# SJTU-ViSYS-team/VisFly

Hardware: AMD Instinct MI355X
Metric: agent-steps/sec (dynamics.step, visual=False) (higher is better)
Workload: dtype f32

## Files before the change

### visfly_amd/csrc/vf_common.hpp

```cpp
#pragma once
#include <hip/hip_runtime.h>

#include <cstdarg>
#include <cstdio>
#include <cstdlib>

#include "visfly_amd.h"

namespace vf {

char* err_buf();

inline int fail(int code, const char* fmt, ...)
{
    va_list ap;
    va_start(ap, fmt);
    vsnprintf(err_buf(), 512, fmt, ap);
    va_end(ap);
    return code;
}

#ifdef VF_CHAIN_PLUGIN
#define VF_HIP(expr)                                                                        \
    do {                                                                                    \
        hipError_t e_ = (expr);                                                             \
        if (e_ != hipSuccess) return -1000 - (int)e_;                                       \
    } while (0)
#else
#define VF_HIP(expr)                                                                        \
    do {                                                                                    \
        hipError_t e_ = (expr);                                                             \
        if (e_ != hipSuccess)                                                               \
            return vf::fail(VF_EHIP, "%s failed: %s (%s:%d)", #expr, hipGetErrorString(e_), \
                            __FILE__, __LINE__);                                            \
    } while (0)
#endif

inline hipStream_t as_stream(vf_stream_t s) { return reinterpret_cast<hipStream_t>(s); }

constexpr int kBlock = 256;

inline int blocks_for(int n) { return (n + kBlock - 1) / kBlock; }

inline int grid_for(long n, int cap = 512)
{
    long b = (n + kBlock - 1) / kBlock;
    return (int)(b < 1 ? 1 : (b > cap ? cap : b));
}

inline bool use_split(int agents_padded, const vf_dyn_cfg& cfg)
{
    if (cfg.action_type != VF_ACT_THRUST && cfg.action_type != VF_ACT_BODYRATE) return false;
    return agents_padded <= 32768;
}

struct vf_env_dev {
    vf_env_cfg cfg;
    unsigned agent0;
    float hit_y;
};

#ifdef __HIPCC__
__device__ __forceinline__ unsigned env_agent0(const vf_env_cfg& e) { return reinterpret_cast<const vf_env_dev&>(e).agent0; }
__device__ __forceinline__ float env_hit_y(const vf_env_cfg& e) { return reinterpret_cast<const vf_env_dev&>(e).hit_y; }

__device__ __forceinline__ double wave_sum(double x)
{
#pragma unroll
    for (int o = 32; o > 0; o >>= 1) x += __shfl_down(x, o, 64);
    return x;
}
__device__ __forceinline__ float wave_sumf(float x)
{
#pragma unroll
    for (int o = 32; o > 0; o >>= 1) x += __shfl_down(x, o, 64);
    return x;
}

struct U4 {
    unsigned x, y, z, w;
};

__device__ __forceinline__ U4 philox4x32_10(U4 ctr, unsigned k0, unsigned k1)
{
#pragma unroll
    for (int r = 0; r < 10; ++r) {
        const unsigned hi0 = __umulhi(0xD2511F53u, ctr.x), lo0 = 0xD2511F53u * ctr.x;
        const unsigned hi1 = __umulhi(0xCD9E8D57u, ctr.z), lo1 = 0xCD9E8D57u * ctr.z;
        ctr = U4{hi1 ^ ctr.y ^ k0, lo1, hi0 ^ ctr.w ^ k1, lo0};
        k0 += 0x9E3779B9u;
        k1 += 0xBB67AE85u;
    }
    return ctr;
}

__device__ __forceinline__ float u01(unsigned x) { return (float)(x & 0xFFFFFFu) * (1.0f / 16777216.0f); }

constexpr unsigned kTagPpoNoise = 0xac7u, kTagRowNoise = 0xb977u;

__device__ __forceinline__ void philox_normal4(unsigned row, unsigned long long step, unsigned tag, unsigned long long seed, float* e)
{
    const U4 r = philox4x32_10(U4{row, (unsigned)step, (unsigned)(step >> 32), tag}, (unsigned)seed, (unsigned)(seed >> 32));
    const float u1 = ((float)(r.x >> 8) + 1.0f) * (1.0f / 16777216.0f), u2 = (float)(r.y >> 8) * (1.0f / 16777216.0f);
    const float u3 = ((float)(r.z >> 8) + 1.0f) * (1.0f / 16777216.0f), u4 = (float)(r.w >> 8) * (1.0f / 16777216.0f);
    const float ra = sqrtf(-2.0f * logf(u1)), rb = sqrtf(-2.0f * logf(u3));
    const float two_pi = 6.28318530717958647692f;
    e[0] = ra * cosf(two_pi * u2); e[1] = ra * sinf(two_pi * u2); e[2] = rb * cosf(two_pi * u4); e[3] = rb * sinf(two_pi * u4);
}

__device__ __forceinline__ float act_fwd(float z, int kind)
{
    switch (kind) {
    case VF_ACTIVATION_RELU: return z > 0.0f ? z : 0.0f;
// ... 123 lines not shown
```

### visfly_amd/csrc/vf_dyn_device.hpp

```cpp
#pragma once
#include <hip/hip_runtime.h>

#include "vf_common.hpp"
#include "vf_pair_algebra.hpp"
#include "vf_step_consts.hpp"
#include "vf_xmath.hpp"
#include "visfly_amd.h"

#pragma clang fp contract(off)

namespace vf {

struct Agent {
    float p[3];
    Quat q;
    float v[3];
    float w[3];
    float wm[4];
    float T[4];
    float aa[3];
    float acc[3];
    float t;
    float wnd[3];
};


__device__ __forceinline__ float clampf(float v, float lo, float hi)
{
    float r = v < lo ? lo : v;
    return r > hi ? hi : r;
}

struct RotorK {
    vf_f2 K0, K1;
};
__device__ __forceinline__ RotorK rotor_k(const vf_dyn_cfg& c)
{
    RotorK k{pair_of(c.c_motor, c.tm0), pair_of(c.tm1, c.tm2)};
    keep_in_vgprs(k.K0);
    keep_in_vgprs(k.K1);
    return k;
}

struct IntervalMats {
    Mat4P B;
    Mat3P J, Jinv;
    RotorK k;
};
__device__ __forceinline__ IntervalMats interval_mats(const vf_dyn_cfg& c)
{
    return IntervalMats{mat4_pairs(c.B), mat3_pairs(c.J), mat3_pairs(c.Jinv), rotor_k(c)};
}

struct MatsOfCfg {
    static constexpr bool paired_sqrt = false;
    __device__ __forceinline__ IntervalMats operator()(const vf_dyn_cfg& c) const { return interval_mats(c); }
};
struct StepConstsV {
    float4 v[8];
};
__device__ __forceinline__ StepConstsV load_step_consts(const vf_dyn_cfg* cp)
{
    unsigned z;
    asm("v_mov_b32 %0, 0" : "=v"(z));
    const float4* p = reinterpret_cast<const float4*>(reinterpret_cast<const char*>(cp) + kStepConstsOffset + z);
    StepConstsV k;
#pragma unroll
    for (int j = 0; j < 8; ++j) k.v[j] = p[j];
    return k;
}
struct MatsOfBlock {
    static constexpr bool paired_sqrt = true;
    StepConstsV k;
    __device__ __forceinline__ IntervalMats operator()(const vf_dyn_cfg& c) const
    {
        IntervalMats M;
#pragma unroll
        for (int j = 0; j < 4; ++j) {
            M.B.c01[j] = pair_of(k.v[j].x, k.v[j].y);
            M.B.c23[j] = pair_of(k.v[j].z, k.v[j].w);
        }
        const vf_f2 h[8] = {pair_of(k.v[4].x, k.v[4].y), pair_of(k.v[4].z, k.v[4].w), pair_of(k.v[5].x, k.v[5].y), pair_of(k.v[5].z, k.v[5].w),
                            pair_of(k.v[6].x, k.v[6].y), pair_of(k.v[6].z, k.v[6].w), pair_of(k.v[7].x, k.v[7].y), pair_of(k.v[7].z, k.v[7].w)};
#pragma unroll
        for (int j = 0; j < 3; ++j) {
            M.J.r0[j] = c.J[j];
            M.Jinv.r0[j] = c.Jinv[j];
            M.J.c12[j] = h[j];
            M.Jinv.c12[j] = h[3 + j];
        }
        M.k.K0 = h[6];
        M.k.K1 = h[7];
#pragma unroll
        for (int j = 0; j < 4; ++j) { keep_in_vgprs(M.B.c01[j]); keep_in_vgprs(M.B.c23[j]); }
#pragma unroll
        for (int j = 0; j < 3; ++j) { keep_in_vgprs(M.J.c12[j]); keep_in_vgprs(M.Jinv.c12[j]); }
        keep_in_vgprs(M.k.K0);
        keep_in_vgprs(M.k.K1);
        return M;
    }
};

struct Vec3P {
    float x;
    vf_f2 yz;
};

__device__ __forceinline__ void derivs(const IntervalMats& M, const QuatP& q, const QuatP& wq, const vf_f2 ft01, const vf_f2 ft23,
                                       QuatP& dq, Vec3P& dw)
{
    const QuatP p = qmul_p<false, false>(q, wq);
    const vf_f2 half = {0.5f, 0.5f};
    dq.wx = p.wx * half;
    dq.yz = p.yz * half;
    float Jw0;
    vf_f2 Jw12;
    mat3_p(M.J, wq.wx, wq.yz, Jw0, Jw12);
    const float w0 = wq.wx[1], w1 = wq.yz[0], w2 = wq.yz[1];
    const float c0 = __builtin_fmaf(w1, Jw12[1], -(w2 * Jw12[0]));
    const float c1 = __builtin_fmaf(w2, Jw0, -(w0 * Jw12[1]));
    const float c2 = __builtin_fmaf(w0, Jw12[0], -(w1 * Jw0));
    vf_f2 d0p = ft01;
    d0p[1] = ft01[1] - c0;
    const vf_f2 d12 = {ft23[0] - c1, ft23[1] - c2};
    mat3_p(M.Jinv, d0p, d12, dw.x, dw.yz);
}
// ... 397 lines not shown
struct NoCheckpoint {
    __device__ __forceinline__ void head(int, const Agent&) const {}
    __device__ __forceinline__ void end(const Agent&) const {}
};

struct RotorsP {
    vf_f2 Td[2], wd[2], wm[2], T[2];
    __device__ __forceinline__ RotorsP(const Agent& s, const float* Td_, const float* wd_)
    {
#pragma unroll
        for (int h = 0; h < 2; ++h) {
            Td[h] = pair_of(Td_[2 * h], Td_[2 * h + 1]);
            wd[h] = pair_of(wd_[2 * h], wd_[2 * h + 1]);
            wm[h] = pair_of(s.wm[2 * h], s.wm[2 * h + 1]);
            T[h] = pair_of(s.T[2 * h], s.T[2 * h + 1]);
        }
    }
    __device__ __forceinline__ void store(Agent& s) const
    {
#pragma unroll
        for (int h = 0; h < 2; ++h) {
            s.wm[2 * h] = wm[h][0]; s.wm[2 * h + 1] = wm[h][1];
            s.T[2 * h] = T[h][0]; s.T[2 * h + 1] = T[h][1];
        }
    }
};

template <int ACT, int INTEG, bool CTRL_DELAY, class CK = NoCheckpoint>
__device__ __forceinline__ void control_interval(const vf_dyn_cfg& c, Agent& s, const float* a,
                                                 const float* kl, const float* kq, bool vstrided = false, const CK& ck = CK{})
{
    float Td[4], wd[4];
    desired_thrusts<ACT>(c, s, a, Td, vstrided);
    rotor_setpoint<CTRL_DELAY>(c, Td, wd);
#pragma unroll 1
    for (int sub = 0; sub < c.interval_steps; ++sub) {
        ck.head(sub, s);
        float ft[4];
        motor_substep<CTRL_DELAY>(c, Td, wd, s.wm, s.T, ft);
        trans_substep<INTEG>(c, s.q, ft[0], kl, kq, s.wnd, s.p, s.v, s.acc);
        rot_substep<INTEG>(c, ft + 1, s.q, s.w, s.aa);
    }
    ck.end(s);
    finish_interval(c, s);
}

template <int ACT, int INTEG, bool CTRL_DELAY, class CK = NoCheckpoint, class MF = MatsOfCfg>
__device__ __forceinline__ void control_interval_pairs(const vf_dyn_cfg& c, Agent& s, const float* a,
                                                 const float* kl, const float* kq, bool vstrided = false, const CK& ck = CK{},
                                                 const MF& mf = MF{})
{
    float Td[4], wd[4];
    desired_thrusts<ACT>(c, s, a, Td, vstrided);
    rotor_setpoint<CTRL_DELAY, MF::paired_sqrt>(c, Td, wd);
    const IntervalMats M = mf(c);
    RotorsP r(s, Td, wd);
    QuatP q = to_pairs(s.q), wq{pair_of(0.0f, s.w[0]), pair_of(s.w[1], s.w[2])};
    const auto mirror = [&] {
        r.store(s);
        s.q = to_quat(q);
        s.w[0] = wq.wx[1]; s.w[1] = wq.yz[0]; s.w[2] = wq.yz[1];
    };
    const SubstepCfg sc = substep_cfg(c);
#pragma unroll 1
    for (int sub = 0; sub < sc.interval_steps; ++sub) {
        if constexpr (!__is_same(CK, NoCheckpoint)) {
            if (sub != 0) mirror();
            ck.head(sub, s);
        }
        vf_f2 ft01, ft23;
        motor_substep<CTRL_DELAY>(M.k, M.B, r.Td, r.wd, r.wm, r.T, ft01, ft23);
        trans_substep<INTEG>(sc, q, ft01[0], kl, kq, s.wnd, s.p, s.v, s.acc);
        rot_substep<INTEG>(sc, M, ft01, ft23, q, wq, s.aa);
    }
    mirror();
    ck.end(s);
    finish_interval(c, s);
}

typedef float vf_f4 __attribute__((ext_vector_type(4)));

template <int MODE>
__device__ __forceinline__ void st4_mode(float4* p, const float4 v)
{
    if constexpr (MODE == 0) {
        *p = v;
    } else {
        const vf_f4 x = {v.x, v.y, v.z, v.w};
        if constexpr (MODE == 1) asm volatile("global_store_dwordx4 %0, %1, off sc1" : : "v"(p), "v"(x) : "memory");
        else if constexpr (MODE == 2) asm volatile("global_store_dwordx4 %0, %1, off nt" : : "v"(p), "v"(x) : "memory");
        else asm volatile("global_store_dwordx4 %0, %1, off sc0 sc1" : : "v"(p), "v"(x) : "memory");
    }
}
template <int MODE>
__device__ __forceinline__ void st1_mode(float* p, const float v)
{
    if constexpr (MODE == 0) *p = v;
    else if constexpr (MODE == 1) asm volatile("global_store_dword %0, %1, off sc1" : : "v"(p), "v"(v) : "memory");
    else if constexpr (MODE == 2) asm volatile("global_store_dword %0, %1, off nt" : : "v"(p), "v"(v) : "memory");
    else asm volatile("global_store_dword %0, %1, off sc0 sc1" : : "v"(p), "v"(v) : "memory");
}

__device__ __forceinline__ float4* granule(float* __restrict__ S, int G, int i, int g)
{
    return reinterpret_cast<float4*>(S) + ((size_t)(i >> 6) * G + g) * VF_TILE + (i & 63);
}
// ... 249 lines not shown
```

### visfly_amd/csrc/vf_env.hip

```cpp
#include "vf_env_epilogue.hpp"

#pragma clang fp contract(off)

#ifdef VF_ENV_TRACE
__device__ unsigned long long* vf_env_trace_buf = nullptr;
__device__ unsigned vf_env_trace_cnt = 0, vf_env_trace_cap = 0;
extern "C" int vf_debug_env_trace(unsigned long long* buf, unsigned cap)
{
    unsigned zero = 0;
    if (hipMemcpyToSymbol(HIP_SYMBOL(vf_env_trace_buf), &buf, sizeof(buf)) != hipSuccess) return -1;
    if (hipMemcpyToSymbol(HIP_SYMBOL(vf_env_trace_cnt), &zero, sizeof(zero)) != hipSuccess) return -1;
    if (hipMemcpyToSymbol(HIP_SYMBOL(vf_env_trace_cap), &cap, sizeof(cap)) != hipSuccess) return -1;
    return 0;
}
#define VF_TR(i) tr[i] = __builtin_amdgcn_s_memrealtime()
#else
#define VF_TR(i)
#endif

namespace vf {

template <int KIND, int ACT, int INTEG, bool CTRL_DELAY, bool LAZY_SLOT = false, bool STRAIGHT = false>
__global__ __launch_bounds__(kBlock) void k_env_step(const vf_dyn_cfg* __restrict__ cp, const vf_env_cfg* __restrict__ ep, float* S,
                                                     const float4* action, int N, int G, int head, int helper, int delay_steps,
                                                     int g_drag, const EnvArgs g0)
{
    const vf_dyn_cfg& c = *cp;
    const vf_env_cfg& e = *ep;
    __shared__ __attribute__((aligned(16))) float tile[kBlock * 13];
    EnvArgs g = g0;
    g.d.S = S; g.d.action = action; g.d.N = N; g.d.G = G; g.d.head = head; g.helper = helper; g.d.g_drag = g_drag;
    if constexpr (STRAIGHT) {
        static_assert(!LAZY_SLOT, "the straight-line instance loads the spawn slot eagerly");
        g.d.g_drag = -1; g.d.wind = nullptr;
        g.out.done_list = nullptr; g.out.done_count = nullptr;
        g.stale = nullptr; g.auto_reset = 1;
        __builtin_assume(g.helper > 0);
        __builtin_assume(g.g_spawn_rd >= 0);
    }
    if (g.helper != 0 && (int)blockIdx.x >= g.helper) {
        const int nbm = g.helper;
        const int base = ((int)blockIdx.x - nbm) * kHelperSpan * kBlock + (int)threadIdx.x;
#pragma unroll 1
        for (int k = 0; k < kHelperSpan; ++k) spawn_helper(e, g, base + k * kBlock);
        return;
    }
#ifdef VF_ENV_TRACE
    unsigned long long tr[13];
#endif
    VF_TR(0);
    const int i = blockIdx.x * kBlock + threadIdx.x;
    const bool live = i < g.d.N;
    Agent s;
    Spares sp;
    float a[4], head_bits = 0.0f;
    ring_exchange_d(g.d, i, live, head_bits, a, nullptr, delay_steps);
    load_agent<false>(g.d.S, g.d.G, i, s, sp);
    float4 dk0 = make_float4(0.f, 0.f, 0.f, 0.f), dk1 = dk0;
    if (g.d.g_drag >= 0) { dk0 = *granule(g.d.S, g.d.G, i, g.d.g_drag); dk1 = *granule(g.d.S, g.d.G, i, g.d.g_drag + 1); }
    StepConstsV kv;
    if constexpr (STRAIGHT) kv = load_step_consts(cp);
#ifdef VF_ENV_TRACE
    VF_TR(1);
    prefetch_const_lines<(sizeof(vf_dyn_cfg) + 63) / 64, 2>(cp, ep, &ep->obs_mode);
    VF_TR(2);
    prefetch_kernarg<sizeof(EnvArgs) + 56>();
    VF_TR(3);
#else
    prefetch_kernarg_and_const_lines<sizeof(EnvArgs) + 56, (sizeof(vf_dyn_cfg) + 63) / 64, 2>(cp, ep, &ep->obs_mode);
#endif
    load_wind(c, g.d, i, live, s);
    if (delay_steps > 0) sp.vel = head_bits;
    float kl[3], kq[3];
    if (g.d.g_drag >= 0) {
        kl[0] = dk0.y; kl[1] = dk0.z; kl[2] = dk0.w;
        kq[0] = dk1.y; kq[1] = dk1.z; kq[2] = dk1.w;
    } else {
#pragma unroll
        for (int k = 0; k < 3; ++k) { kl[k] = c.k_lin[k]; kq[k] = c.k_quad[k]; }
    }
    if constexpr (STRAIGHT)
        asm("" : "+v"(s.wnd[0]), "+v"(s.wnd[1]), "+v"(s.wnd[2]), "+v"(kl[0]), "+v"(kl[1]), "+v"(kl[2]), "+v"(kq[0]), "+v"(kq[1]), "+v"(kq[2]));
#ifdef VF_ENV_TRACE
    asm volatile("s_waitcnt vmcnt(0)" ::: "memory");
    VF_TR(4);
    struct TraceCk {
        unsigned long long* tr;
        __device__ __forceinline__ void head(int sub, const Agent& s) const
        {
            if (sub < 2) { asm volatile("" :: "v"(s.wm[0]), "v"(s.q.w) : "memory"); tr[5 + sub] = __builtin_amdgcn_s_memrealtime(); }
        }
        __device__ __forceinline__ void end(const Agent&) const {}
    };
    control_interval_pairs<ACT, INTEG, CTRL_DELAY>(c, s, a, kl, kq, g.d.vstrided != 0, TraceCk{tr});
    asm volatile("" :: "v"(s.p[0]), "v"(s.q.w), "v"(s.v[0]), "v"(s.w[0]) : "memory");
    VF_TR(7);
#else
    if constexpr (STRAIGHT)
        control_interval_pairs<ACT, INTEG, CTRL_DELAY, NoCheckpoint, MatsOfBlock>(c, s, a, kl, kq, g.d.vstrided != 0, NoCheckpoint{}, MatsOfBlock{kv});
    else
        control_interval_pairs<ACT, INTEG, CTRL_DELAY>(c, s, a, kl, kq, g.d.vstrided != 0);
#endif
    const int wave = threadIdx.x >> 6;
#ifdef VF_ENV_TRACE
    env_epilogue<KIND, true, 1, false, LAZY_SLOT, STRAIGHT ? 7 : 0>(c, e, g, i, live, s, sp, blockIdx.x * kBlock + wave * 64, tile + wave * 64 * 13, nullptr, nullptr, tr);
    asm volatile("" ::: "memory");
    VF_TR(11);
    asm volatile("s_waitcnt vmcnt(0)" ::: "memory");
    VF_TR(12);
    if ((threadIdx.x & 63) == 0 && vf_env_trace_buf) {
        const unsigned slot = atomicAdd(&vf_env_trace_cnt, 1u);
        if (slot < vf_env_trace_cap) {
            unsigned long long* o = vf_env_trace_buf + (size_t)slot * 16;
            for (int k = 0; k < 13; ++k) o[k] = tr[k];
            o[13] = ((unsigned long long)blockIdx.x << 8) | wave;
            unsigned xcc = 0;
            asm volatile("s_getreg_b32 %0, hwreg(HW_REG_XCC_ID)" : "=s"(xcc));
            unsigned hwid = 0;
            asm volatile("s_getreg_b32 %0, hwreg(HW_REG_HW_ID)" : "=s"(hwid));
            o[14] = ((unsigned long long)xcc << 32) | hwid;
        }
    }
#else
    env_epilogue<KIND, true, 1, false, LAZY_SLOT, STRAIGHT ? 7 : 0>(c, e, g, i, live, s, sp, blockIdx.x * kBlock + wave * 64, tile + wave * 64 * 13);
#endif
}



template <int KIND>
__global__ __launch_bounds__(kBlock) void k_env_finish(const vf_dyn_cfg* __restrict__ cp, const vf_env_cfg* __restrict__ ep, const EnvArgs g)
{
    const vf_dyn_cfg& c = *cp;
    const vf_env_cfg& e = *ep;
    __shared__ __attribute__((aligned(16))) float tile[kBlock * 13];
    const int i = blockIdx.x * kBlock + threadIdx.x;
    const bool live = i < g.d.N;
    Agent s;
    Spares sp;
    load_agent<false>(g.d.S, g.d.G, i, s, sp);
    load_wind(c, g.d, i, live, s);
    const int wave = threadIdx.x >> 6;
    env_epilogue<KIND, true, 1, true>(c, e, g, i, live, s, sp, blockIdx.x * kBlock + wave * 64, tile + wave * 64 * 13);
}

template <int KIND, int ACT, int INTEG, bool CTRL_DELAY>
__global__ __launch_bounds__(kBlock) void k_env_rollout(const vf_dyn_cfg* __restrict__ cp, const vf_env_cfg* __restrict__ ep, const EnvArgs g0)
{
    const vf_dyn_cfg& c = *cp;
    const vf_env_cfg& e = *ep;
    __shared__ __attribute__((aligned(16))) float tile[kBlock * 13];
    const int i = blockIdx.x * kBlock + threadIdx.x;
    const int wave = threadIdx.x >> 6;
    EnvArgs g = g0;
    const bool live = i < g.d.N;
    Agent s;
    Spares sp;
    float a[4], head_bits = 0.0f;
    ring_exchange(c, g.d, i, live, head_bits, a);
    load_agent<false>(g.d.S, g.d.G, i, s, sp);
    load_wind(c, g.d, i, live, s);
    for (int k = 0;;) {
        if (c.delay_steps > 0) sp.vel = head_bits;
        float kl[3], kq[3];
        drag_of(c, g.d, i, kl, kq);
        control_interval_pairs<ACT, INTEG, CTRL_DELAY>(c, s, a, kl, kq, g.d.vstrided != 0);
        env_epilogue<KIND, false>(c, e, g, i, live, s, sp, blockIdx.x * kBlock + wave * 64, tile + wave * 64 * 13);
        if (++k >= g.K) break;
        g.d.action += g.action_stride;
        g.out.obs += g.obs_stride;
        g.out.reward += g.reward_stride;
        g.out.done += g.done_stride;
        g.d.head = g.d.head + 1 == c.delay_steps ? 0 : g.d.head + 1;
        ring_exchange(c, g.d, i, live, head_bits, a);
    }
    store_agent(g.d.S, g.d.G, i, s, sp);
}
// ... 612 lines not shown
```

### visfly_amd/csrc/vf_env_epilogue.hpp

```cpp
#pragma once
#include "vf_env_device.hpp"
#include "vf_handles.hpp"

#pragma clang fp contract(off)

namespace vf {

struct EnvArgs {
    DynArgs d;
    vf_env_out out;
    int g_race;
    int auto_reset;
    int K = 1;
    long long action_stride = 0, obs_stride = 0, reward_stride = 0, done_stride = 0;
    const float* ext_point = nullptr;
    const unsigned char* ext_oob = nullptr;
    int g_spawn_rd = -1, g_spawn_wr = -1, helper = 0;
    unsigned long long* stale = nullptr;
    int n_tiles = 0, stale_wr = 0;
};

struct EnvRegs {
    int step_count;
    float rewards;
// ... 14 lines not shown
__device__ __forceinline__ int set_flag(int flags, int bit, bool on) { return on ? (flags | bit) : (flags & ~bit); }

__device__ __forceinline__ int collision_flags(int flags, const Collision& col)
{
    flags = set_flag(flags, VF_F_COLLISION, col.hit);
    flags = set_flag(flags, VF_F_OUT_BOUNDS, col.oob);
    if (col.hit) flags |= VF_F_ONCE_COLLIDED;
    return flags;
}

struct SpawnSlot {
    float4 g0, g1, g2, g3;
};

#ifndef VF_HELPER_SPAN
#define VF_HELPER_SPAN 1
#endif
constexpr int kHelperSpan = VF_HELPER_SPAN;

__device__ __forceinline__ void spawn_helper(const vf_env_cfg& e, const EnvArgs& g, int i)
{
    if (i >= g.d.N) return;
    unsigned long long* word = nullptr;
    if (g.stale) {
        word = g.stale + (size_t)g.stale_wr * g.n_tiles + (i >> 6);
        if (!((*word >> (i & 63)) & 1ull)) return;
    }
    const unsigned need = ((unsigned)__float_as_int(granule(g.d.S, g.d.G, i, VF_G_ACC)->x) >> 8) + 1u;
    float4* dst = granule(g.d.S, g.d.G, i, g.g_spawn_wr);
    if (__float_as_uint(dst->x) != need) {
        Agent s;
        spawn_agent(e, env_agent0(e), i, need, true, s);
        const int gs = 64;
        dst[0] = make_float4(__uint_as_float(need), s.p[0], s.p[1], s.p[2]);
        dst[gs] = make_float4(s.q.w, s.q.x, s.q.y, s.q.z);
        dst[2 * gs] = make_float4(s.t, s.v[0], s.v[1], s.v[2]);
        dst[3 * gs] = make_float4(0.0f, s.w[0], s.w[1], s.w[2]);
    }
    if (word) atomicAnd(word, ~(1ull << (i & 63)));
}

__device__ __forceinline__ SpawnSlot load_spawn_slot(const EnvArgs& g, int i, bool wanted = true)
{
    const float4* src = granule(g.d.S, g.d.G, i, (wanted && g.g_spawn_rd >= 0) ? g.g_spawn_rd : 0);
    SpawnSlot slot;
    slot.g0 = src[0]; slot.g1 = src[64]; slot.g2 = src[128]; slot.g3 = src[192];
    return slot;
}

template <int KIND, bool STORE_STATE = true, int LANES = 1, bool EXT = false, bool LAZY_SLOT = false, int STRAIGHT = 0>
__device__ __forceinline__ void env_epilogue(const vf_dyn_cfg& c, const vf_env_cfg& e, const EnvArgs& g, int i, bool live,
                                             Agent& s, Spares& sp, int wave_first, float* tile, float* reward_reg = nullptr,
                                             bool* done_reg = nullptr, unsigned long long* tr = nullptr,
                                             int* gate_reg = nullptr)
{
#ifdef VF_ENV_TRACE
#define VF_EPI_TR(k, x) do { if (tr) { asm volatile("" :: "v"(x) : "memory"); tr[k] = __builtin_amdgcn_s_memrealtime(); } } while (0)
#else
#define VF_EPI_TR(k, x)
#endif
    EnvRegs er = unpack_env(sp);
    const float vel[3] = {s.v[0] + s.wnd[0], s.v[1] + s.wnd[1], s.v[2] + s.wnd[2]};
    constexpr bool NO_ROOT = (STRAIGHT & 4) && KIND == VF_ENV_HOVER && !EXT;
    Collision col = bbox_collision<NO_ROOT>(e, s.p);
    if constexpr (EXT) {
        if (g.ext_point && live) {
            const float* q = g.ext_point + 3 * (size_t)i;
#pragma unroll
            for (int d = 0; d < 3; ++d) { col.cp[d] = q[d]; col.vec[d] = q[d] - s.p[d]; }
            col.dis = norm3(col.vec[0], col.vec[1], col.vec[2]);
            col.hit = col.dis < e.uav_radius;
        }
        if (g.ext_oob && live) col.oob = g.ext_oob[i] != 0;
    }
    er.flags = collision_flags(er.flags, col);
    er.step_count += 1;

    bool success = false, failure = false;
    if constexpr (KIND == VF_ENV_NAV) {
        success = norm3(s.p[0] - e.target[0], s.p[1] - e.target[1], s.p[2] - e.target[2]) <= e.success_radius;
        if (e.reward_mode == VF_REWARD_NAV2) failure = col.hit;
    }
    bool ep_done = (er.flags & VF_F_EPISODE_DONE) || success || failure || (er.flags & VF_F_OUT_BOUNDS);
    if (e.is_collision_reset) ep_done = ep_done || (er.flags & VF_F_COLLISION);
    const bool truncated = er.step_count >= e.max_episode_steps;
    const bool done = ep_done || truncated;
    SpawnSlot slot;
    const bool use_slot = done && g.auto_reset && g.g_spawn_rd >= 0;
    if constexpr (!LAZY_SLOT) {
        const bool wave_ends = __builtin_amdgcn_ballot_w64(use_slot) != 0;
        slot = load_spawn_slot(g, i, wave_ends);
    } else {
        if (use_slot) slot = load_spawn_slot(g, i);
    }
    float reward;
    int gate = 0, passed = 0, gate_pre = 0;
    float4 race = make_float4(0.f, 0.f, 0.f, 0.f);
    if constexpr (KIND == VF_ENV_HOVER) {
        reward = hover_reward<(STRAIGHT & 2) != 0>(s.p, e.target, s.q, vel, s.w);
    } else if constexpr (KIND == VF_ENV_NAV) {
        if (e.reward_mode == VF_REWARD_NAV2) {
            reward = nav2_reward(e, s.p, vel, s.w, success);
        } else {
            reward = nav_reward(e, s.p, s.q, vel, s.w, col, success, er.step_count, c.trig_mode);
        }
    } else {
        race = *granule(g.d.S, g.d.G, i, g.g_race);
        gate = __float_as_int(race.x);
        gate = (unsigned)gate < (unsigned)e.n_gates ? gate : 0;
        gate_pre = gate;
        passed = __float_as_int(race.y);
        const float* gt = e.gates[gate];
        const bool pass = norm3(s.p[0] - gt[0], s.p[1] - gt[1], s.p[2] - gt[2]) <= e.success_radius;
        gate = gate + (pass ? 1 : 0);
        gate = gate == e.n_gates ? 0 : gate;
        passed += pass ? 1 : 0;
        reward = hover_reward(s.p, e.gates[gate], s.q, vel, s.w);
        reward = reward + (pass ? 1.0f : 0.0f) * 20.0f;
        race.z = __int_as_float(pass ? 1 : 0);
    }
    VF_EPI_TR(8, reward);
    er.rewards = er.rewards + reward;
    er.flags = set_flag(er.flags, VF_F_EPISODE_DONE, ep_done);
    er.flags = set_flag(er.flags, VF_F_SUCCESS, success);
    er.flags = set_flag(er.flags, VF_F_FAILURE, failure);
    er.flags = set_flag(er.flags, VF_F_DONE, done);
    if (g.out.done_list) {
        const bool mine = live && done && (LANES == 1 || (threadIdx.x & (LANES - 1)) == 0);
        const unsigned long long m = __ballot(mine);
        if (m) {
            const int lane = threadIdx.x & 63, first = __ffsll((long long)m) - 1;
            int base = 0;
            if (lane == first) base = atomicAdd(g.out.done_count, __popcll(m));
            base = __shfl(base, first);
            if (mine) g.out.done_list[base + __popcll(m & ((1ull << lane) - 1ull))] = i;
        }
    }
    float o[13];
    obs_row(c, s, o);
    if constexpr (!(STRAIGHT & 1)) obs_variant(e, o);
    if (live) {
        g.out.reward[i] = reward;
        if (reward_reg) *reward_reg = reward;
        if (done_reg) *done_reg = done;
        g.out.done[i] = done ? 1 : 0;
        if (done) {
            if (g.out.ep_return) g.out.ep_return[i] = er.rewards;
            if (g.out.ep_length) g.out.ep_length[i] = er.step_count;
            if (g.out.ep_flags)
                g.out.ep_flags[i] = (success ? VF_EP_SUCCESS : 0) | (truncated ? VF_EP_TRUNCATED : 0) |
                                    ((er.flags & VF_F_ONCE_COLLIDED) ? VF_EP_COLLIDED : 0) |
                                    (ep_done ? VF_EP_EPISODE_DONE : 0);
            if constexpr (kind_is_racing(KIND)) {
                if (g.out.ep_past_gates) g.out.ep_past_gates[i] = passed;
                if (g.out.terminal_gate) g.out.terminal_gate[i] = gate_pre;
            }
            if (g.out.terminal_obs) {
                if constexpr (KIND == VF_ENV_RACING2) {
                    float ot[16];
                    race2_obs(e, o, gate_pre, ot);
                    float* to = g.out.terminal_obs + 16 * (size_t)i;
#pragma unroll
                    for (int k = 0; k < 16; ++k) to[k] = ot[k];
                } else {
                    float* to = g.out.terminal_obs + 13 * (size_t)i;
#pragma unroll
                    for (int k = 0; k < 13; ++k) to[k] = o[k];
                }
            }
        }
    }
    if (g.stale) {
        const unsigned long long ending = __builtin_amdgcn_ballot_w64(done && g.auto_reset != 0 && live);
        if (ending && (threadIdx.x & 63) == 0) {
            atomicOr(g.stale + (i >> 6), ending);
            atomicOr(g.stale + g.n_tiles + (i >> 6), ending);
        }
    }
    if (done && g.auto_reset) {
        unsigned episode = ((unsigned)er.flags >> 8) + 1u;
        if constexpr (kind_is_racing(KIND)) {
            gate = racing_choose_gate(s.p);
            passed = 0;
            race.z = __int_as_float(0);
        }
        if (use_slot && __float_as_uint(slot.g0.x) == episode) {
            s.p[0] = slot.g0.y; s.p[1] = slot.g0.z; s.p[2] = slot.g0.w;
            s.q = Quat{slot.g1.x, slot.g1.y, slot.g1.z, slot.g1.w};
            s.t = slot.g2.x;
            s.v[0] = slot.g2.y; s.v[1] = slot.g2.z; s.v[2] = slot.g2.w;
            s.w[0] = slot.g3.y; s.w[1] = slot.g3.z; s.w[2] = slot.g3.w;
        } else {
            spawn_agent(e, env_agent0(e), i, episode, true, s);
        }
        reset_rotors(c, s);
        for (int q = 0; q < c.delay_steps; ++q)
            *granule(g.d.S, g.d.G, i, VF_G_RING + q) = make_float4(0.f, 0.f, 0.f, 0.f);
        if (g.d.g_drag >= 0 && e.drag_random > 0.0f) {
            float4 kl4, kq4;
            spawn_drag(c, e, env_agent0(e), i, episode, kl4, kq4);
            *granule(g.d.S, g.d.G, i, g.d.g_drag) = kl4;
            *granule(g.d.S, g.d.G, i, g.d.g_drag + 1) = kq4;
        }
        col = bbox_collision<NO_ROOT>(e, s.p);
        er.flags = (int)(episode << 8);
        er.flags = set_flag(er.flags, VF_F_COLLISION, col.hit);
        er.flags = set_flag(er.flags, VF_F_OUT_BOUNDS, col.oob);
        er.step_count = 0;
        er.rewards = 0.0f;
        obs_row(c, s, o);
        if constexpr (!(STRAIGHT & 1)) obs_variant(e, o);
    }
    if constexpr (kind_is_racing(KIND)) {
        race.x = __int_as_float(gate);
        race.y = __int_as_float(passed);
        *granule(g.d.S, g.d.G, i, g.g_race) = race;
        if (live && g.out.gate) g.out.gate[i] = gate;
        if (gate_reg) *gate_reg = gate;
    }
    pack_env(er, sp);
    VF_EPI_TR(9, sp.acc);
    if constexpr (STORE_STATE) store_agent(g.d.S, g.d.G, i, s, sp);
    VF_EPI_TR(10, sp.acc);
    if constexpr (KIND == VF_ENV_RACING2) {
        float o16[16];
        race2_obs(e, o, gate, o16);
        if constexpr (LANES == 4) store_rows_quads<16>(g.out.obs, g.d.N, wave_first, o16, tile);
        else store_rows_coalesced<16>(g.out.obs, g.d.N, wave_first, o16, tile);
    } else if constexpr (LANES == 4) store_rows_quads<13>(g.out.obs, g.d.N, wave_first, o, tile);
    else store_rows_coalesced<13>(g.out.obs, g.d.N, wave_first, o, tile);
}

}
```

### visfly_amd/csrc/vf_handles.hpp

```cpp
#pragma once
#include "vf_common.hpp"
#include "vf_step_consts.hpp"

struct vf_dyn {
    vf_dyn_cfg cfg;
    int N, Npad, G, g_drag, g_extra;
    float* S = nullptr;
    long long tick = 0;
    int vel_strided = 0;
    vf_dyn_cfg* d_cfg = nullptr;
    struct vf_env_cfg* d_env_dummy = nullptr;
    const float* wind = nullptr;
};

struct vf_env {
    vf_dyn dyn;
    vf_env_cfg cfg;
    int g_race;
    int g_spawn = -1;
    unsigned long long* d_stale = nullptr;
    int stale_all = 1;
    vf_env_cfg* d_cfg = nullptr;
    unsigned agent0 = 0;
};

namespace vf {

inline int check_dyn_cfg(const vf_dyn_cfg* cfg)
{
    if (cfg->action_type < VF_ACT_THRUST || cfg->action_type > VF_ACT_POSITION)
        return fail(VF_EINVAL, "action_type %d not supported (thrust=0, bodyrate=1, velocity=2, position=3)",
                    cfg->action_type);
    if (cfg->integrator != VF_INT_EULER && cfg->integrator != VF_INT_RK4)
        return fail(VF_EINVAL, "integrator %d not supported (euler=0, rk4=1)", cfg->integrator);
    if (cfg->interval_steps <= 0 || cfg->delay_steps < 0 || cfg->delay_steps > 64)
        return fail(VF_EINVAL, "bad interval_steps/delay_steps");
    return VF_OK;
}

inline void init_dyn_handle(vf_dyn* h, const vf_dyn_cfg* cfg, int N, int per_agent_drag, int extra)
{
    h->cfg = *cfg;
    h->N = N;
    h->Npad = (N + kBlock - 1) / kBlock * kBlock;
    h->g_drag = per_agent_drag ? VF_G_FIXED + cfg->delay_steps : -1;
    h->g_extra = VF_G_FIXED + cfg->delay_steps + (per_agent_drag ? 2 : 0);
    h->G = h->g_extra + extra;
    h->S = nullptr;
    h->tick = 0;
    h->vel_strided = 0;
}

template <class T>
inline int upload_cfg(const T& host, T** dev)
{
    VF_HIP(hipMalloc(reinterpret_cast<void**>(dev), sizeof(T)));
    VF_HIP(hipMemcpy(*dev, &host, sizeof(T), hipMemcpyHostToDevice));
    return VF_OK;
}
inline int upload_dyn_dev(const vf_dyn_cfg& cfg, vf_dyn_cfg** dev)
{
    vf_dyn_dev host{};
    host.cfg = cfg;
    pack_step_consts(cfg, &host.k);
    if (!*dev) VF_HIP(hipMalloc(reinterpret_cast<void**>(dev), sizeof(vf_dyn_dev)));
    VF_HIP(hipMemcpy(*dev, &host, sizeof(vf_dyn_dev), hipMemcpyHostToDevice));
    return VF_OK;
}
inline int upload_env_dev(const vf_env_cfg& cfg, unsigned agent0, vf_env_cfg** dev)
{
    const vf_env_dev host{cfg, agent0, hit_threshold(cfg.uav_radius)};
    if (!*dev) VF_HIP(hipMalloc(reinterpret_cast<void**>(dev), sizeof(vf_env_dev)));
    VF_HIP(hipMemcpy(*dev, &host, sizeof(vf_env_dev), hipMemcpyHostToDevice));
    return VF_OK;
}
template <class T>
inline void release_cfg(T** dev)
{
    if (*dev) (void)hipFree(*dev);
    *dev = nullptr;
}

inline int ring_head(const vf_dyn* h, int ahead = 0)
{
    return h->cfg.delay_steps > 0 ? (int)((h->tick + ahead) % h->cfg.delay_steps) : 0;
}

inline int refuse_capture(const vf_dyn* h, hipStream_t st, const char* who)
{
    if (h->cfg.delay_steps <= 1) return VF_OK;
    hipStreamCaptureStatus cs = hipStreamCaptureStatusNone;
    if (hipStreamIsCapturing(st, &cs) != hipSuccess) {
        (void)hipGetLastError();
        return VF_OK;
    }
    if (cs != hipStreamCaptureStatusNone)
        return fail(VF_ESTATE, "%s: the stream is capturing and delay_steps = %d: a captured launch bakes ONE delay-ring slot "
                               "into the graph (every replay would reuse it).  Use vf_env_graph_create / vf_env_graph_launch",
                    who, h->cfg.delay_steps);
    return VF_OK;
}

inline int set_ring_phase(vf_dyn* h, int phase, const char* who)
{
    const int D = h->cfg.delay_steps;
    if (phase < 0 || (D > 0 ? phase >= D : phase != 0)) return fail(VF_EINVAL, "%s: phase %d outside [0, %d)", who, phase, D > 0 ? D : 1);
    h->tick = phase;
    return VF_OK;
}

}
```

### visfly_amd/csrc/vf_step_consts.hpp

```cpp
#pragma once
#include <cmath>
#include <cstddef>
#include <cstdint>
#include <cstring>

#include "visfly_amd.h"

namespace vf {

struct vf_step_consts {
    float Bcol[4][4];
    float J12[3][2];
    float Jinv12[3][2];
    float K0[2], K1[2];
};
static_assert(sizeof(vf_step_consts) == 128, "eight 16-byte loads");

constexpr size_t kStepConstsOffset = (sizeof(vf_dyn_cfg) + 63) / 64 * 64;
struct vf_dyn_dev {
    vf_dyn_cfg cfg;
    alignas(64) vf_step_consts k;
};
static_assert(offsetof(vf_dyn_dev, k) == kStepConstsOffset, "the kernels address the block by this offset");

inline void pack_step_consts(const vf_dyn_cfg& c, vf_step_consts* out)
{
    for (int k = 0; k < 4; ++k)
        for (int r = 0; r < 4; ++r) out->Bcol[k][r] = c.B[4 * r + k];
    for (int k = 0; k < 3; ++k) {
        out->J12[k][0] = c.J[3 + k];
        out->J12[k][1] = c.J[6 + k];
        out->Jinv12[k][0] = c.Jinv[3 + k];
        out->Jinv12[k][1] = c.Jinv[6 + k];
    }
    out->K0[0] = c.c_motor; out->K0[1] = c.tm0;
    out->K1[0] = c.tm1; out->K1[1] = c.tm2;
}

inline float hit_threshold(float r)
{
    if (r != r) return r;
    if (!(r > 0.0f)) return 0.0f;
    if (std::isinf(r)) return r;
    uint32_t lo = 0u, hi = 0x7f800000u;
    while (lo < hi) {
        const uint32_t mid = lo + (hi - lo) / 2;
        float y;
        std::memcpy(&y, &mid, 4);
        if (std::sqrt(y) >= r) hi = mid;
        else lo = mid + 1;
    }
    float T;
    std::memcpy(&T, &hi, 4);
    return T;
}

}
```

Measured before the change: 7.137 billion.

## Pack hot dynamics and env scalars into aligned blocks loaded as wide scalar loads

Adds packed, line-aligned scalar-constant blocks to the device-side dynamics and env configs. The straight-line env-step kernel now loads them with a few wide 16-dword scalar loads into a local config copy instead of issuing scattered field loads. The limit and env-epilogue constants are deferred until after desired thrusts are computed, so their latency overlaps compute. This aims to cut scalar-memory latency and load count in the kernel prologue, at the cost of extra SGPR pressure, a larger device config and duplicated packing code that must stay in sync.

```diff
diff --git a/visfly_amd/csrc/vf_common.hpp b/visfly_amd/csrc/vf_common.hpp
--- a/visfly_amd/csrc/vf_common.hpp
+++ b/visfly_amd/csrc/vf_common.hpp
@@ -5,6 +5,7 @@
 #include <cstdio>
 #include <cstdlib>
 
+#include "vf_step_consts.hpp"
 #include "visfly_amd.h"
 
 namespace vf {
@@ -54,11 +55,6 @@
     return agents_padded <= 32768;
 }
 
-struct vf_env_dev {
-    vf_env_cfg cfg;
-    unsigned agent0;
-    float hit_y;
-};
 
 #ifdef __HIPCC__
 __device__ __forceinline__ unsigned env_agent0(const vf_env_cfg& e) { return reinterpret_cast<const vf_env_dev&>(e).agent0; }
diff --git a/visfly_amd/csrc/vf_dyn_device.hpp b/visfly_amd/csrc/vf_dyn_device.hpp
--- a/visfly_amd/csrc/vf_dyn_device.hpp
+++ b/visfly_amd/csrc/vf_dyn_device.hpp
@@ -53,7 +53,7 @@
 }
 
 struct MatsOfCfg {
-    static constexpr bool paired_sqrt = false;
+    static constexpr bool paired_sqrt = false, late_loads = false;
     __device__ __forceinline__ IntervalMats operator()(const vf_dyn_cfg& c) const { return interval_mats(c); }
 };
 struct StepConstsV {
@@ -69,9 +69,78 @@
     for (int j = 0; j < 8; ++j) k.v[j] = p[j];
     return k;
 }
+typedef unsigned vf_u16 __attribute__((ext_vector_type(16)));
+typedef unsigned vf_u8 __attribute__((ext_vector_type(8)));
+struct ScalarConstsV {
+    float4 binvT[4], air[3];
+};
+__device__ __forceinline__ void load_consts_v(const vf_dyn_cfg* cp, StepConstsV& k, ScalarConstsV& sv)
+{
+    unsigned z;
+    asm("v_mov_b32 %0, 0" : "=v"(z));
+    const float4* p = reinterpret_cast<const float4*>(reinterpret_cast<const char*>(cp) + kStepConstsOffset + z);
+#pragma unroll
+    for (int j = 0; j < 8; ++j) k.v[j] = p[j];
+    const float4* q = reinterpret_cast<const float4*>(reinterpret_cast<const char*>(cp) + kScalarConstsOffset + kScalarBinvT + z);
+#pragma unroll
+    for (int j = 0; j < 4; ++j) sv.binvT[j] = q[j];
+#pragma unroll
+    for (int j = 0; j < 3; ++j) sv.air[j] = q[4 + j];
+}
+__device__ __forceinline__ void load_scalar_consts(const vf_dyn_cfg* cp, const ScalarConstsV& sv, vf_dyn_cfg& lc)
+{
+    const char* b = reinterpret_cast<const char*>(cp) + kScalarConstsOffset;
+    vf_u16 s0 = *reinterpret_cast<const vf_u16*>(b + kScalarS0), s1 = *reinterpret_cast<const vf_u16*>(b + kScalarS1),
+           s2 = *reinterpret_cast<const vf_u16*>(b + kScalarS2);
+    asm volatile("" : "+s"(s0), "+s"(s1), "+s"(s2));
+    const auto f = [](unsigned u) { return __uint_as_float(u); };
+    lc.acc_half = f(s0[0]); lc.acc_mean = f(s0[1]); lc.rate_half = f(s0[2]); lc.rate_mean = f(s0[3]);
+    lc.m = f(s0[4]); lc.T_init = f(s0[5]); lc.w_init = f(s0[6]); lc.one_minus_c = f(s0[7]);
+    lc.rot_tm1sq = f(s0[8]); lc.rot_4tm0 = f(s0[9]); lc.tm2 = f(s0[10]); lc.rot_scale = f(s0[11]);
+    lc.rot_neg_tm1 = f(s0[12]); lc.dt = f(s0[13]); lc.g_z = f(s0[14]); lc.interval_steps = (int)s0[15];
+#pragma unroll
+    for (int k = 0; k < 9; ++k) {
+        lc.JP[k] = f(s1[k]);
+        lc.J[k] = k < 7 ? f(s1[9 + k]) : f(s2[k - 7]);
+        lc.Dm[k] = f(s2[2 + k]);
+    }
+#pragma unroll
+    for (int k = 0; k < 3; ++k) lc.Jinv[k] = f(s2[11 + k]);
+#pragma unroll
+    for (int k = 0; k < 4; ++k) {
+        lc.Binv[k] = sv.binvT[k].x; lc.Binv[4 + k] = sv.binvT[k].y; lc.Binv[8 + k] = sv.binvT[k].z; lc.Binv[12 + k] = sv.binvT[k].w;
+    }
+    lc.k_lin[0] = sv.air[0].x; lc.k_quad[0] = sv.air[0].y; lc.k_lin[1] = sv.air[0].z; lc.k_lin[2] = sv.air[0].w;
+    lc.wind[0] = sv.air[1].x; lc.wind[1] = sv.air[1].y; lc.k_quad[1] = sv.air[1].z; lc.k_quad[2] = sv.air[1].w;
+    lc.wind[2] = sv.air[2].x; lc.T_min = sv.air[2].y; lc.T_max = sv.air[2].z;
+}
+struct LateConsts {
+    const vf_dyn_cfg* cp;
+    const vf_env_cfg* ep;
+    vf_dyn_cfg* lc;
+    vf_env_dev* le;
+    __device__ __forceinline__ void load(const float* after) const
+    {
+        unsigned off = 0;
+        asm volatile("" : "+s"(off) : "v"(after[0]), "v"(after[1]), "v"(after[2]), "v"(after[3]));
+        const vf_u8 lim = *reinterpret_cast<const vf_u8*>(reinterpret_cast<const char*>(cp) + kScalarConstsOffset + kScalarLim + off);
+        const vf_u16 ek = *reinterpret_cast<const vf_u16*>(reinterpret_cast<const char*>(ep) + kEnvScalarsOffset + off);
+        const auto f = [](unsigned u) { return __uint_as_float(u); };
+        lc->ctrl_dt = f(lim[0]); lc->pos_xy_lim = f(lim[1]); lc->pos_z_lo = f(lim[2]); lc->pos_z_hi = f(lim[3]);
+        lc->vel_lim = f(lim[4]); lc->omg_lim = f(lim[5]); lc->trig_mode = (int)lim[6];
+        vf_env_cfg& e = le->cfg;
+        e.max_episode_steps = (int)ek[0]; e.is_collision_reset = (int)ek[1]; e.reward_mode = (int)ek[2];
+        le->hit_y = f(ek[3]);
+#pragma unroll
+        for (int k = 0; k < 3; ++k) { e.bbox_lo[k] = f(ek[4 + k]); e.bbox_hi[k] = f(ek[7 + k]); e.target[k] = f(ek[10 + k]); }
+        e.success_radius = f(ek[13]); e.uav_radius = f(ek[14]);
+    }
+};
+
 struct MatsOfBlock {
-    static constexpr bool paired_sqrt = true;
+    static constexpr bool paired_sqrt = true, late_loads = true;
     StepConstsV k;
+    LateConsts late;
     __device__ __forceinline__ IntervalMats operator()(const vf_dyn_cfg& c) const
     {
         IntervalMats M;
@@ -575,6 +644,7 @@
 {
     float Td[4], wd[4];
     desired_thrusts<ACT>(c, s, a, Td, vstrided);
+    if constexpr (MF::late_loads) mf.late.load(Td);
     rotor_setpoint<CTRL_DELAY, MF::paired_sqrt>(c, Td, wd);
     const IntervalMats M = mf(c);
     RotorsP r(s, Td, wd);
diff --git a/visfly_amd/csrc/vf_env.hip b/visfly_amd/csrc/vf_env.hip
--- a/visfly_amd/csrc/vf_env.hip
+++ b/visfly_amd/csrc/vf_env.hip
@@ -25,7 +25,14 @@
                                                      const float4* action, int N, int G, int head, int helper, int delay_steps,
                                                      int g_drag, const EnvArgs g0)
 {
-    const vf_dyn_cfg& c = *cp;
+    vf_dyn_cfg lc;
+    vf_env_dev le;
+    if constexpr (STRAIGHT) {
+        lc = *cp;
+        lc.delay_steps = delay_steps;
+        le = *reinterpret_cast<const vf_env_dev*>(ep);
+    }
+    const vf_dyn_cfg& c = STRAIGHT ? lc : *cp;
     const vf_env_cfg& e = *ep;
     __shared__ __attribute__((aligned(16))) float tile[kBlock * 13];
     EnvArgs g = g0;
@@ -59,7 +66,8 @@
     float4 dk0 = make_float4(0.f, 0.f, 0.f, 0.f), dk1 = dk0;
     if (g.d.g_drag >= 0) { dk0 = *granule(g.d.S, g.d.G, i, g.d.g_drag); dk1 = *granule(g.d.S, g.d.G, i, g.d.g_drag + 1); }
     StepConstsV kv;
-    if constexpr (STRAIGHT) kv = load_step_consts(cp);
+    ScalarConstsV sv;
+    if constexpr (STRAIGHT) load_consts_v(cp, kv, sv);
 #ifdef VF_ENV_TRACE
     VF_TR(1);
     prefetch_const_lines<(sizeof(vf_dyn_cfg) + 63) / 64, 2>(cp, ep, &ep->obs_mode);
@@ -67,7 +75,8 @@
     prefetch_kernarg<sizeof(EnvArgs) + 56>();
     VF_TR(3);
 #else
-    prefetch_kernarg_and_const_lines<sizeof(EnvArgs) + 56, (sizeof(vf_dyn_cfg) + 63) / 64, 2>(cp, ep, &ep->obs_mode);
+    if constexpr (STRAIGHT) load_scalar_consts(cp, sv, lc);
+    else prefetch_kernarg_and_const_lines<sizeof(EnvArgs) + 56, (sizeof(vf_dyn_cfg) + 63) / 64, 2>(cp, ep, &ep->obs_mode);
 #endif
     load_wind(c, g.d, i, live, s);
     if (delay_steps > 0) sp.vel = head_bits;
@@ -97,7 +106,8 @@
     VF_TR(7);
 #else
     if constexpr (STRAIGHT)
-        control_interval_pairs<ACT, INTEG, CTRL_DELAY, NoCheckpoint, MatsOfBlock>(c, s, a, kl, kq, g.d.vstrided != 0, NoCheckpoint{}, MatsOfBlock{kv});
+        control_interval_pairs<ACT, INTEG, CTRL_DELAY, NoCheckpoint, MatsOfBlock>(c, s, a, kl, kq, g.d.vstrided != 0, NoCheckpoint{},
+                                                                                  MatsOfBlock{kv, LateConsts{cp, ep, &lc, &le}});
     else
         control_interval_pairs<ACT, INTEG, CTRL_DELAY>(c, s, a, kl, kq, g.d.vstrided != 0);
 #endif
@@ -122,7 +132,8 @@
         }
     }
 #else
-    env_epilogue<KIND, true, 1, false, LAZY_SLOT, STRAIGHT ? 7 : 0>(c, e, g, i, live, s, sp, blockIdx.x * kBlock + wave * 64, tile + wave * 64 * 13);
+    env_epilogue<KIND, true, 1, false, LAZY_SLOT, STRAIGHT ? 7 : 0>(c, e, g, i, live, s, sp, blockIdx.x * kBlock + wave * 64, tile + wave * 64 * 13,
+                                                                    nullptr, nullptr, nullptr, nullptr, STRAIGHT ? &le.cfg : nullptr);
 #endif
 }
 
diff --git a/visfly_amd/csrc/vf_env_epilogue.hpp b/visfly_amd/csrc/vf_env_epilogue.hpp
--- a/visfly_amd/csrc/vf_env_epilogue.hpp
+++ b/visfly_amd/csrc/vf_env_epilogue.hpp
@@ -90,8 +90,10 @@
 __device__ __forceinline__ void env_epilogue(const vf_dyn_cfg& c, const vf_env_cfg& e, const EnvArgs& g, int i, bool live,
                                              Agent& s, Spares& sp, int wave_first, float* tile, float* reward_reg = nullptr,
                                              bool* done_reg = nullptr, unsigned long long* tr = nullptr,
-                                             int* gate_reg = nullptr)
-{
+                                             int* gate_reg = nullptr,
+                                             const vf_env_cfg* hot = nullptr)
+{
+    const vf_env_cfg& eh = hot ? *hot : e;
 #ifdef VF_ENV_TRACE
 #define VF_EPI_TR(k, x) do { if (tr) { asm volatile("" :: "v"(x) : "memory"); tr[k] = __builtin_amdgcn_s_memrealtime(); } } while (0)
 #else
@@ -100,7 +102,7 @@
     EnvRegs er = unpack_env(sp);
     const float vel[3] = {s.v[0] + s.wnd[0], s.v[1] + s.wnd[1], s.v[2] + s.wnd[2]};
     constexpr bool NO_ROOT = (STRAIGHT & 4) && KIND == VF_ENV_HOVER && !EXT;
-    Collision col = bbox_collision<NO_ROOT>(e, s.p);
+    Collision col = bbox_collision<NO_ROOT>(eh, s.p);
     if constexpr (EXT) {
         if (g.ext_point && live) {
             const float* q = g.ext_point + 3 * (size_t)i;
@@ -116,12 +118,12 @@
 
     bool success = false, failure = false;
     if constexpr (KIND == VF_ENV_NAV) {
-        success = norm3(s.p[0] - e.target[0], s.p[1] - e.target[1], s.p[2] - e.target[2]) <= e.success_radius;
-        if (e.reward_mode == VF_REWARD_NAV2) failure = col.hit;
+        success = norm3(s.p[0] - eh.target[0], s.p[1] - eh.target[1], s.p[2] - eh.target[2]) <= eh.success_radius;
+        if (eh.reward_mode == VF_REWARD_NAV2) failure = col.hit;
     }
     bool ep_done = (er.flags & VF_F_EPISODE_DONE) || success || failure || (er.flags & VF_F_OUT_BOUNDS);
-    if (e.is_collision_reset) ep_done = ep_done || (er.flags & VF_F_COLLISION);
-    const bool truncated = er.step_count >= e.max_episode_steps;
+    if (eh.is_collision_reset) ep_done = ep_done || (er.flags & VF_F_COLLISION);
+    const bool truncated = er.step_count >= eh.max_episode_steps;
     const bool done = ep_done || truncated;
     SpawnSlot slot;
     const bool use_slot = done && g.auto_reset && g.g_spawn_rd >= 0;
@@ -135,12 +137,12 @@
     int gate = 0, passed = 0, gate_pre = 0;
     float4 race = make_float4(0.f, 0.f, 0.f, 0.f);
     if constexpr (KIND == VF_ENV_HOVER) {
-        reward = hover_reward<(STRAIGHT & 2) != 0>(s.p, e.target, s.q, vel, s.w);
+        reward = hover_reward<(STRAIGHT & 2) != 0>(s.p, eh.target, s.q, vel, s.w);
     } else if constexpr (KIND == VF_ENV_NAV) {
-        if (e.reward_mode == VF_REWARD_NAV2) {
-            reward = nav2_reward(e, s.p, vel, s.w, success);
+        if (eh.reward_mode == VF_REWARD_NAV2) {
+            reward = nav2_reward(eh, s.p, vel, s.w, success);
         } else {
-            reward = nav_reward(e, s.p, s.q, vel, s.w, col, success, er.step_count, c.trig_mode);
+            reward = nav_reward(eh, s.p, s.q, vel, s.w, col, success, er.step_count, c.trig_mode);
         }
     } else {
         race = *granule(g.d.S, g.d.G, i, g.g_race);
@@ -240,7 +242,7 @@
             *granule(g.d.S, g.d.G, i, g.d.g_drag) = kl4;
             *granule(g.d.S, g.d.G, i, g.d.g_drag + 1) = kq4;
         }
-        col = bbox_collision<NO_ROOT>(e, s.p);
+        col = bbox_collision<NO_ROOT>(eh, s.p);
         er.flags = (int)(episode << 8);
         er.flags = set_flag(er.flags, VF_F_COLLISION, col.hit);
         er.flags = set_flag(er.flags, VF_F_OUT_BOUNDS, col.oob);
diff --git a/visfly_amd/csrc/vf_handles.hpp b/visfly_amd/csrc/vf_handles.hpp
--- a/visfly_amd/csrc/vf_handles.hpp
+++ b/visfly_amd/csrc/vf_handles.hpp
@@ -60,16 +60,16 @@
 }
 inline int upload_dyn_dev(const vf_dyn_cfg& cfg, vf_dyn_cfg** dev)
 {
-    vf_dyn_dev host{};
-    host.cfg = cfg;
-    pack_step_consts(cfg, &host.k);
+    vf_dyn_dev host;
+    fill_dyn_dev(cfg, &host);
     if (!*dev) VF_HIP(hipMalloc(reinterpret_cast<void**>(dev), sizeof(vf_dyn_dev)));
     VF_HIP(hipMemcpy(*dev, &host, sizeof(vf_dyn_dev), hipMemcpyHostToDevice));
     return VF_OK;
 }
 inline int upload_env_dev(const vf_env_cfg& cfg, unsigned agent0, vf_env_cfg** dev)
 {
-    const vf_env_dev host{cfg, agent0, hit_threshold(cfg.uav_radius)};
+    vf_env_dev host;
+    fill_env_dev(cfg, agent0, &host);
     if (!*dev) VF_HIP(hipMalloc(reinterpret_cast<void**>(dev), sizeof(vf_env_dev)));
     VF_HIP(hipMemcpy(*dev, &host, sizeof(vf_env_dev), hipMemcpyHostToDevice));
     return VF_OK;
diff --git a/visfly_amd/csrc/vf_step_consts.hpp b/visfly_amd/csrc/vf_step_consts.hpp
--- a/visfly_amd/csrc/vf_step_consts.hpp
+++ b/visfly_amd/csrc/vf_step_consts.hpp
@@ -16,12 +16,37 @@
 };
 static_assert(sizeof(vf_step_consts) == 128, "eight 16-byte loads");
 
+struct vf_scalar_consts {
+    float acc_half, acc_mean, rate_half, rate_mean;
+    float m, T_init, w_init, one_minus_c;
+    float rot_tm1sq, rot_4tm0, tm2, rot_scale;
+    float rot_neg_tm1, dt, g_z;
+    int32_t interval_steps;
+    float JP[9], J[9], Dm[9], Jinv0[3];
+    float pad_s2[2];
+    float ctrl_dt, pos_xy_lim, pos_z_lo, pos_z_hi, vel_lim, omg_lim;
+    int32_t trig_mode;
+    float pad_lim;
+    float BinvT[4][4];
+    float air[3][4];
+    float pad_end[4];
+};
+static_assert(sizeof(vf_scalar_consts) == 352, "5.5 lines");
+constexpr size_t kScalarS0 = 0, kScalarS1 = 64, kScalarS2 = 128, kScalarLim = 192, kScalarBinvT = 224, kScalarAir = 288;
+static_assert(offsetof(vf_scalar_consts, JP) == kScalarS1 && offsetof(vf_scalar_consts, J) + 7 * 4 == kScalarS2 &&
+              offsetof(vf_scalar_consts, ctrl_dt) == kScalarLim && offsetof(vf_scalar_consts, BinvT) == kScalarBinvT &&
+              offsetof(vf_scalar_consts, air) == kScalarAir, "the offsets the kernels load from");
+static_assert(kScalarBinvT % 16 == 0 && kScalarAir % 16 == 0, "16-byte vector loads");
+
 constexpr size_t kStepConstsOffset = (sizeof(vf_dyn_cfg) + 63) / 64 * 64;
+constexpr size_t kScalarConstsOffset = kStepConstsOffset + sizeof(vf_step_consts);
 struct vf_dyn_dev {
     vf_dyn_cfg cfg;
     alignas(64) vf_step_consts k;
+    alignas(64) vf_scalar_consts s;
 };
 static_assert(offsetof(vf_dyn_dev, k) == kStepConstsOffset, "the kernels address the block by this offset");
+static_assert(offsetof(vf_dyn_dev, s) == kScalarConstsOffset, "the kernels address the scalar half by this offset");
 
 inline void pack_step_consts(const vf_dyn_cfg& c, vf_step_consts* out)
 {
@@ -35,6 +60,33 @@
     }
     out->K0[0] = c.c_motor; out->K0[1] = c.tm0;
     out->K1[0] = c.tm1; out->K1[1] = c.tm2;
+}
+
+inline void pack_scalar_consts(const vf_dyn_cfg& c, vf_scalar_consts* out)
+{
+    std::memset(out, 0, sizeof *out);
+    out->acc_half = c.acc_half; out->acc_mean = c.acc_mean; out->rate_half = c.rate_half; out->rate_mean = c.rate_mean;
+    out->m = c.m; out->T_init = c.T_init; out->w_init = c.w_init; out->one_minus_c = c.one_minus_c;
+    out->rot_tm1sq = c.rot_tm1sq; out->rot_4tm0 = c.rot_4tm0; out->tm2 = c.tm2; out->rot_scale = c.rot_scale;
+    out->rot_neg_tm1 = c.rot_neg_tm1; out->dt = c.dt; out->g_z = c.g_z; out->interval_steps = c.interval_steps;
+    for (int k = 0; k < 9; ++k) { out->JP[k] = c.JP[k]; out->J[k] = c.J[k]; out->Dm[k] = c.Dm[k]; }
+    for (int k = 0; k < 3; ++k) out->Jinv0[k] = c.Jinv[k];
+    out->trig_mode = c.trig_mode;
+    out->ctrl_dt = c.ctrl_dt; out->pos_xy_lim = c.pos_xy_lim; out->pos_z_lo = c.pos_z_lo; out->pos_z_hi = c.pos_z_hi;
+    out->vel_lim = c.vel_lim; out->omg_lim = c.omg_lim;
+    for (int k = 0; k < 4; ++k)
+        for (int r = 0; r < 4; ++r) out->BinvT[k][r] = c.Binv[4 * r + k];
+    out->air[0][0] = c.k_lin[0]; out->air[0][1] = c.k_quad[0]; out->air[0][2] = c.k_lin[1]; out->air[0][3] = c.k_lin[2];
+    out->air[1][0] = c.wind[0]; out->air[1][1] = c.wind[1]; out->air[1][2] = c.k_quad[1]; out->air[1][3] = c.k_quad[2];
+    out->air[2][0] = c.wind[2]; out->air[2][1] = c.T_min; out->air[2][2] = c.T_max;
+}
+
+inline void fill_dyn_dev(const vf_dyn_cfg& c, vf_dyn_dev* out)
+{
+    std::memset(static_cast<void*>(out), 0, sizeof *out);
+    out->cfg = c;
+    pack_step_consts(c, &out->k);
+    pack_scalar_consts(c, &out->s);
 }
 
 inline float hit_threshold(float r)
@@ -55,4 +107,35 @@
     return T;
 }
 
+struct vf_env_scalars {
+    int32_t max_episode_steps, is_collision_reset, reward_mode;
+    float hit_y;
+    float bbox_lo[3], bbox_hi[3];
+    float target[3];
+    float success_radius, uav_radius;
+    float pad;
+};
+static_assert(sizeof(vf_env_scalars) == 64, "one 16-dword load");
+struct vf_env_dev {
+    vf_env_cfg cfg;
+    unsigned agent0;
+    float hit_y;
+    alignas(64) vf_env_scalars k;
+};
+constexpr size_t kEnvScalarsOffset = (sizeof(vf_env_cfg) + 8 + 63) / 64 * 64;
+static_assert(offsetof(vf_env_dev, k) == kEnvScalarsOffset, "the kernels address the env scalars by this offset");
+
+inline void fill_env_dev(const vf_env_cfg& c, unsigned agent0, vf_env_dev* out)
+{
+    std::memset(static_cast<void*>(out), 0, sizeof *out);
+    out->cfg = c;
+    out->agent0 = agent0;
+    out->hit_y = hit_threshold(c.uav_radius);
+    vf_env_scalars& k = out->k;
+    k.max_episode_steps = c.max_episode_steps; k.is_collision_reset = c.is_collision_reset; k.reward_mode = c.reward_mode;
+    k.hit_y = out->hit_y;
+    for (int d = 0; d < 3; ++d) { k.bbox_lo[d] = c.bbox_lo[d]; k.bbox_hi[d] = c.bbox_hi[d]; k.target[d] = c.target[d]; }
+    k.success_radius = c.success_radius; k.uav_radius = c.uav_radius;
 }
+
+}
```

Result: no change. 7.137 billion (median of 2 runs) (+0.0%).
